# princeton-computational-imaging/Neural-Volume-Super-Resolution

Hardware: AMD Instinct MI355X
Metric: rendered rays/sec (64+128 samples) at 800x800 Lego-like view (higher is better)
Workload: dtype f32 as 2 f16 limbs (3 MFMA products, f32 acc); 1 GPU; Blender-'lego'-like 800x800 view, 64 coarse + 128 fine samples, tri-plane decoder (3x800^2x48 + 32^2x48 planes, 4+4x128 MLP), 1 view per GPU per step; partition=view

## Files before the change

include/nvsr.h:

```cpp
#ifndef NVSR_H
#define NVSR_H
#include <stdint.h>

#ifdef __cplusplus
extern "C" {
#endif

typedef void* nvsr_stream_t;

typedef enum {
    NVSR_OK = 0,
    NVSR_ERR_SHAPE = 1,
    NVSR_ERR_LAUNCH = 2,
    NVSR_ERR_NULL = 3,
    NVSR_ERR_ALIGN = 4
} nvsr_status;

#define NVSR_PLANE_CHANNELS 48
#define NVSR_DEC_CHANNELS 128
#define NVSR_DEC_LAYERS 4
#define NVSR_DECODER_NATURAL_FLOATS 130564
#define NVSR_DECODER_PACKED_F32_FLOATS 130576
#define NVSR_DECODER_PACKED_FLOATS 453136
#define NVSR_DECODER_PACKED_BWD_FLOATS 487424

typedef struct nvsr_scene {
    const float* planes[4];
    int32_t ph[4], pw[4];
    float lo[5];
    float range[5];
    float proj[3][6];
} nvsr_scene;

int nvsr_version(void);

#define NVSR_ARITH_INHERIT (-1)
#define NVSR_ARITH_INVALID (-2)
#define NVSR_ARITH_F32 0
#define NVSR_ARITH_F16 1
#define NVSR_ARITH_F16X2 2
#define NVSR_ARITH_BF16X3 3
#define NVSR_ARITH_DEFAULT NVSR_ARITH_F16X2
int nvsr_get_decoder_arithmetic(void);
int nvsr_set_decoder_arithmetic(int mode);
int nvsr_set_range_flag(uint32_t* device_word);
uint32_t* nvsr_get_range_flag(void);
int nvsr_release_render_scratch(void);
int64_t nvsr_render_scratch_bytes(void);
int nvsr_internal_group_order(const int* trips, int64_t G, int S, int* out, nvsr_stream_t stream);
int nvsr_internal_copy_group_order(int* dst, int64_t G, nvsr_stream_t stream);
int nvsr_internal_live_order(int* live_n, int64_t N, int S, nvsr_stream_t stream);
int nvsr_internal_colour_order_bins(void);
int nvsr_internal_copy_live_counts(int* dst, int64_t N, nvsr_stream_t stream);
int nvsr_internal_point_order(const int* entries, const float* lists, const float* rays, int64_t N, int S, int bands, int* points, int* steps, int* offsets,
                              nvsr_stream_t stream);
int nvsr_internal_point_bands(void);
int nvsr_internal_copy_point_steps(int* dst, int64_t G, nvsr_stream_t stream);
int64_t nvsr_occupancy_words(int G);
int64_t nvsr_occupancy_workspace_floats(int G, int K);
int nvsr_occupancy_build(const nvsr_scene* scene, const float* packed_decoder, int G, int K, float threshold, int dilate, int arithmetic, uint32_t* grid,
                         float* workspace, nvsr_stream_t stream);
int nvsr_render_pass_occupancy_arith(const nvsr_scene* scene, const float* packed_decoder, int64_t N, int S, const float* rays, const float* z, int lindisp,
                                     int white_bkgd, float* rgb, float* disp, float* acc, float* weights, float* depth, const uint32_t* grid, int G, int arithmetic,
                                     nvsr_stream_t stream);
int nvsr_render_rays_occupancy_arith(const nvsr_scene* scene, const float* packed_coarse, const float* packed_fine, int64_t N, int Nc, int Nf,
                                     const float* rays, int lindisp, int white_bkgd, const float* t_rand, const float* u, float* rgb_c, float* disp_c,
                                     float* acc_c, float* rgb_f, float* disp_f, float* acc_f, float* workspace, const uint32_t* grid_coarse, int G_coarse,
                                     const uint32_t* grid_fine, int G_fine, int arithmetic, nvsr_stream_t stream);
int nvsr_internal_occupancy_probes(const nvsr_scene* scene, int G, int K, float* x, nvsr_stream_t stream);
int nvsr_internal_occupancy_cull(const nvsr_scene* scene, int64_t N, int S, const float* rays, const float* z, int lindisp, const uint32_t* grid, int G, int* kept,
                                 int* kept_n, nvsr_stream_t stream);
int nvsr_internal_copy_kept_counts(int* dst, int64_t N, nvsr_stream_t stream);
int nvsr_limb_gemm_probe(int arithmetic, int K, const float* W, const float* X, float* Y, nvsr_stream_t stream);
#define NVSR_CONV_ARITH_DEFAULT NVSR_ARITH_F16X2
int nvsr_get_conv_arithmetic(void);
int nvsr_set_conv_arithmetic(int mode);

int nvsr_plane_to_channel_last(const float* nchw, float* nhwc, int C, int H, int W, nvsr_stream_t stream);
int nvsr_plane_from_channel_last(const float* nhwc, float* nchw, int C, int H, int W, nvsr_stream_t stream);

int nvsr_pack_decoder(const float* natural, float* packed, nvsr_stream_t stream);

int nvsr_get_ray_bundle(int H, int W, double focal_x, double focal_y, const float* c2w, int padding, double offset,
                        float* ro, float* rd, nvsr_stream_t stream);
int nvsr_get_ray_bundle_at(int H, int W, double focal_x, double focal_y, const float* c2w, double offset, int64_t N, const int32_t* row_col,
                           float* ro, float* rd, nvsr_stream_t stream);
int nvsr_sample_pixels(int64_t total, int H, int W, uint64_t key, int64_t first, int64_t n, const float* image, int channels,
                       int32_t* row_col, float* target, nvsr_stream_t stream);
uint64_t nvsr_sample_key(uint64_t seed, uint64_t calls);
int nvsr_sample_pixels_seq(int64_t total, int H, int W, uint64_t* state, int64_t first, int64_t n, const float* image, int channels,
                           int32_t* row_col, float* target, nvsr_stream_t stream);
#define NVSR_MSE_PAIR_MAX_ELEMS (1 << 22)
int nvsr_mse_pair(int64_t n, const float* a, const float* b, const float* target, float* losses, float* g_a, float* g_b, nvsr_stream_t stream);
int nvsr_mse_pair_sum(int64_t n, const float* a, const float* b, const float* target, float* losses3, nvsr_stream_t stream);
int nvsr_mse_pair_backward(int64_t n, const float* a, const float* b, const float* target, const float* scale_a, const float* scale_b, float* g_a,
                           float* g_b, nvsr_stream_t stream);
int nvsr_ndc_rays(int H, int W, double focal, double near_, int64_t N, const float* ro, const float* rd, float* ro_out,
                  float* rd_out, nvsr_stream_t stream);
int nvsr_pack_rays(int64_t N, const float* ro, const float* rd, const float* view_src, double near_, double far_,
                   float* rays, nvsr_stream_t stream);
int nvsr_coarse_z(int64_t N, int Nc, const float* rays, int lindisp, const float* t_rand, float* z, nvsr_stream_t stream);

int nvsr_sample_pdf(int64_t N, int nb, int ns, const float* bins, const float* weights, const float* u, float* samples,
                    nvsr_stream_t stream);
int nvsr_cumprod_exclusive(int64_t N, int n, const float* in, float* out, nvsr_stream_t stream);
int nvsr_cumprod_exclusive_backward(int64_t N, int n, const float* in, const float* out, const float* g_out, float* g_in,
                                    nvsr_stream_t stream);
int nvsr_sort_rows(int64_t N, int n, const float* in, float* out, nvsr_stream_t stream);
int nvsr_importance_resample(int64_t N, int Nc, int Nf, const float* z_coarse, const float* weights, const float* u,
                             float* z_fine, nvsr_stream_t stream);

int nvsr_importance_resample_rays(int64_t N, int Nc, int Nf, const float* rays, int lindisp, const float* weights, const float* u,
                                  float* z_fine, nvsr_stream_t stream);

int nvsr_triplane_decode(const nvsr_scene* scene, const float* packed_decoder, int64_t P, const float* x, float* out,
                         nvsr_stream_t stream);
int nvsr_triplane_decode_arith(const nvsr_scene* scene, const float* packed_decoder, int64_t P, const float* x, float* out, int arithmetic,
                               nvsr_stream_t stream);

int nvsr_composite(int64_t N, int S, const float* raw, const float* z, const float* rd, const float* noise, int white_bkgd,
                   float* rgb, float* disp, float* acc, float* weights, float* depth, nvsr_stream_t stream);

int nvsr_composite_mip(int64_t N, int S, const float* raw, const float* z, const float* rd, const float* noise, int white_bkgd,
                       float* rgb, float* disp, float* acc, float* weights , float* depth ,
                       nvsr_stream_t stream);
int nvsr_composite_rays(int64_t N, int S, const float* raw, const float* z, const float* rays, const float* noise, int white_bkgd,
                        float* rgb, float* disp, float* acc, float* weights, float* depth, nvsr_stream_t stream);

int nvsr_render_pass(const nvsr_scene* scene, const float* packed_decoder, int64_t N, int S, const float* rays, const float* z,
                     const float* noise, int white_bkgd, float* rgb, float* disp, float* acc, float* weights, float* depth,
                     nvsr_stream_t stream);

int nvsr_decode_rays(const nvsr_scene* scene, const float* packed_decoder, int64_t N, int S, const float* rays, const float* z,
                     float* raw, nvsr_stream_t stream);

#define NVSR_FUSED_MIN_RAYS 65536
int64_t nvsr_fused_min_rays(void);
int64_t nvsr_render_workspace_floats(int64_t N, int Nc, int Nf);
int nvsr_render_rays(const nvsr_scene* scene, const float* packed_coarse, const float* packed_fine, int64_t N, int Nc, int Nf,
// ... 275 lines not shown
```

neural-volume-super-resolution_amd/capi.py:

```python
import ctypes as C
import os

import torch

from .build import LIB_PATH as _DEFAULT_LIB_PATH

LIB_PATH = os.environ.get("NVSR_HIP_LIB", _DEFAULT_LIB_PATH)

PLANE_CHANNELS = 48
DEC_CHANNELS = 128
DECODER_NATURAL_FLOATS = 130564
DECODER_PACKED_FLOATS = 453136
DECODER_PACKED_BWD_FLOATS = 487424
MIP_NERF_NATURAL_FLOATS = 81092
MIP_NERF_RECORD_FLOATS = 767
MIP_NERF_GRAD_RECORD_FLOATS = 708
PE_NERF_NATURAL_FLOATS = 81476
PE_NERF_RECORD_FLOATS = 770
PE_NERF_GRAD_RECORD_FLOATS = 708
MSE_PAIR_MAX_ELEMS = 1 << 22

_STATUS = {1: "NVSR_ERR_SHAPE (argument out of the supported range)", 2: "NVSR_ERR_LAUNCH (kernel launch failed)",
           3: "NVSR_ERR_NULL (required pointer is NULL)", 4: "NVSR_ERR_ALIGN (pointer not 16-byte aligned)"}

# ... 78 lines not shown
    "nvsr_conv3x3_packed_floats": ([_i, _i], _i64),
    "nvsr_pack_conv3x3": ([_vp, _i, _i, _vp, _vp], _i),
    "nvsr_conv3x3": ([_vp, _i, _i, _i, _vp, _i, _i, _vp, _vp, _vp], _i),
    "nvsr_edsr_natural_floats": ([_i, _i, _i, _i, _i], _i64),
    "nvsr_edsr_packed_floats": ([_i, _i, _i, _i, _i], _i64),
    "nvsr_pack_edsr": ([_vp, _i, _i, _i, _i, _i, _vp, _vp], _i),
    "nvsr_pack_edsr_arith": ([_vp, _i, _i, _i, _i, _i, _vp, _i, _vp], _i),
    "nvsr_edsr_out_size": ([_i, _i, _i, _i, _ip, _ip], _i),
    "nvsr_edsr_workspace_floats": ([_i, _i, _i, _i, _i], _i64),
    "nvsr_edsr_forward": ([_vp, _i, _i, _i, _vp, _i, _i, _i, _i, _vp, _vp, _vp], _i),
    "nvsr_planes_sr_workspace_floats": ([_i, _i, _i, _i, _i, _i, _i, _fp], _i64),
    "nvsr_planes_sr": ([_vp, _i, _i, _i, _vp, _i, _i, _i, _i, _i, _fp, _vp, _vp, _vp, _vp, _vp], _i),
    "nvsr_render_pass_ex": ([C.POINTER(Scene), _vp, _i64, _i, _vp, _vp, _vp, _i, _vp, _vp, _vp, _vp, _vp, _vp, _vp], _i),
    "nvsr_pack_decoder_bwd": ([_vp, _vp, _vp], _i),
    "nvsr_composite_backward": ([_i64, _i, _vp, _vp, _vp, _vp, _i, _vp, _vp, _vp, _vp], _i),
    "nvsr_composite_backward_mip": ([_i64, _i, _vp, _vp, _vp, _vp, _i, _vp, _vp, _vp, _vp], _i),
    "nvsr_composite_backward_depth": ([_i64, _i, _vp, _vp, _vp, _vp, _i, _vp, _vp, _vp, _i, _vp, _vp], _i),
    "nvsr_composite_backward_rays": ([_i64, _i, _vp, _vp, _vp, _vp, _i, _vp, _vp, _vp, _i, _vp, _vp], _i),
    "nvsr_render_pass_backward": ([C.POINTER(Scene), _vp, _vp, _i64, _i, _vp, _vp, _vp, C.POINTER(C.c_void_p), _vp], _i),
    "nvsr_decode_rays_ex": ([C.POINTER(Scene), _vp, _i64, _i, _vp, _vp, _vp, _vp, _vp, _vp], _i),
    "nvsr_render_pass_backward_gates": ([C.POINTER(Scene), _vp, _vp, _i64, _i, _vp, _vp, _vp, _vp, C.POINTER(C.c_void_p), _vp, _vp, _vp], _i),
    "nvsr_view_grad_workspace_floats": ([_i64, _i], _i64),
    "nvsr_decoder_record_floats": ([_i64, _i], _i64),
    "nvsr_render_pass_backward_ex": ([C.POINTER(Scene), _vp, _vp, _i64, _i, _vp, _vp, _vp, C.POINTER(C.c_void_p), _vp, _vp, _vp], _i),
    "nvsr_decoder_weight_grad": ([_i64, _i, _vp, _vp, _vp], _i),
    "nvsr_edsr_forward_batch": ([_vp, _i, _i, _i, _i, _vp, _i, _i, _i, _i, _vp, _vp, _vp], _i),
    "nvsr_planes_sr_batch": ([C.POINTER(C.c_void_p), _i, _i, _i, _i, _vp, _i, _i, _i, _i, _i, _fp, _vp, _vp, C.POINTER(C.c_void_p), _vp, _vp], _i),
    "nvsr_pack_conv3x3_dgrad": ([_vp, _i, _i, _vp, _vp], _i),
    "nvsr_conv3x3_dgrad": ([_vp, _i, _i, _i, _vp, _i, _vp, _vp], _i),
    "nvsr_conv3x3_wgrad_workspace_floats": ([_i, _i, _i, _i], _i64),
    "nvsr_conv3x3_wgrad": ([_vp, _vp, _i, _i, _i, _i, C.c_float, _vp, _vp, _vp], _i),
    "nvsr_edsr_acts_floats": ([_i, _i, _i, _i, _i, _i, _i], _i64),
    "nvsr_edsr_forward_train": ([_vp, _i, _i, _i, _vp, _i, _i, _i, _i, _vp, _vp, _vp], _i),
    "nvsr_edsr_packed_dgrad_floats": ([_i, _i, _i, _i, _i], _i64),
    "nvsr_pack_edsr_dgrad": ([_vp, _i, _i, _i, _i, _i, _vp, _vp], _i),
    "nvsr_pack_edsr_dgrad_arith": ([_vp, _i, _i, _i, _i, _i, _vp, _i, _vp], _i),
    "nvsr_edsr_backward_workspace_floats": ([_i, _i, _i, _i, _i, _i, _i], _i64),
    "nvsr_edsr_backward": ([_vp, _i, _i, _i, _vp, _vp, _i, _i, _i, _i, _vp, _vp, _vp, _vp, _vp], _i),
    "nvsr_planes_sr_keep_floats": ([_i, _i, _i, _i, _i, _i, _i, _fp], _i64),
    "nvsr_planes_sr_train": ([_vp, _i, _i, _i, _vp, _i, _i, _i, _i, _i, _fp, _vp, _vp, _vp, _vp, _vp, _vp], _i),
    "nvsr_planes_sr_backward_workspace_floats": ([_i, _i, _i, _i, _i, _i, _i, _fp], _i64),
    "nvsr_planes_sr_backward": ([_i, _i, _i, _vp, _vp, _i, _i, _i, _i, _i, _fp, _vp, _vp, _vp, _vp, _vp, _vp], _i),
    "nvsr_generic_decoder_natural_floats": ([C.POINTER(DecoderGeometry)], _i64),
    "nvsr_generic_decode_workspace_floats": ([C.POINTER(DecoderGeometry), _i64], _i64),
    "nvsr_generic_decode": ([C.POINTER(Scene), C.POINTER(DecoderGeometry), _vp, _i64, _vp, _vp, _vp, _vp], _i),
    "nvsr_generic_decode_backward_workspace_floats": ([C.POINTER(DecoderGeometry), _i64], _i64),
    "nvsr_generic_decode_backward": ([C.POINTER(Scene), C.POINTER(DecoderGeometry), _vp, _i64, _vp, _vp, _vp, _vp, _vp, _vp, _vp, _vp, _vp], _i),
    "nvsr_generic_decoder_natural_floats_ext": ([C.POINTER(DecoderGeometry), _i], _i64),
    "nvsr_generic_decode_workspace_floats_ext": ([C.POINTER(DecoderGeometry), _i, _i64], _i64),
    "nvsr_generic_decode_backward_workspace_floats_ext": ([C.POINTER(DecoderGeometry), _i, _i64], _i64),
    "nvsr_generic_decode_ext": ([C.POINTER(SceneExt), C.POINTER(DecoderGeometry), _vp, _i64, _vp, _vp, _vp, _vp, _vp], _i),
    "nvsr_generic_fused_supported": ([C.POINTER(DecoderGeometry), _i], _i),
    "nvsr_generic_decode_fused_ext": ([C.POINTER(SceneExt), C.POINTER(DecoderGeometry), _vp, _i64, _vp, _vp, _vp, _vp], _i),
    "nvsr_generic_packed_floats_ext": ([C.POINTER(DecoderGeometry), _i], _i64),
    "nvsr_pack_generic_decoder_ext": ([C.POINTER(DecoderGeometry), _i, _vp, _vp, _vp], _i),
    "nvsr_generic_fused_supported_arith": ([C.POINTER(DecoderGeometry), _i, _i], _i),
    "nvsr_generic_decode_fused_arith_ext": ([C.POINTER(SceneExt), C.POINTER(DecoderGeometry), _vp, _vp, _i64, _vp, _vp, _vp, _i, _vp], _i),
    "nvsr_generic_decode_fused_density_arith_ext": ([C.POINTER(SceneExt), C.POINTER(DecoderGeometry), _vp, _vp, _i64, _vp, _vp, _vp, _i, _vp], _i),
    "nvsr_generic_decode_fused_colour_arith_ext": ([C.POINTER(SceneExt), C.POINTER(DecoderGeometry), _vp, _vp, _i64, _vp, _vp, _vp, _vp, _i64, _vp, _i,
                                                    _vp], _i),
    "nvsr_generic_live_list_workspace_bytes": ([_i64], _i64),
    "nvsr_generic_live_list": ([_i64, _vp, _vp, _vp, _vp, _vp], _i),
    "nvsr_generic_occupancy_build_ext": ([C.POINTER(SceneExt), C.POINTER(DecoderGeometry), _vp, _vp, _i, _i, C.c_float, _i, _i, _vp, _vp, _vp], _i),
    "nvsr_generic_occupancy_keep": ([C.POINTER(SceneExt), _i64, _vp, _vp, _i, _vp, _vp, _vp], _i),
    "nvsr_generic_decode_fused_density_list_arith_ext": ([C.POINTER(SceneExt), C.POINTER(DecoderGeometry), _vp, _vp, _i64, _vp, _vp, _vp, _vp, _i64, _vp,
                                                          _i, _vp], _i),
    "nvsr_generic_decode_backward_ext": ([C.POINTER(SceneExt), C.POINTER(DecoderGeometry), _vp, _i64, _vp, _vp, _vp, _vp, C.POINTER(C.c_void_p),
                                          _vp, _vp], _i),
    "nvsr_generic_backward_fused_supported": ([C.POINTER(DecoderGeometry), _i], _i),
    "nvsr_generic_decode_backward_fused_ext": ([C.POINTER(SceneExt), C.POINTER(DecoderGeometry), _vp, _i64, _vp, _vp, _vp, C.POINTER(C.c_void_p),
                                                _vp], _i),
    "nvsr_ray_points": ([_i64, _i, _vp, _vp, _vp, _vp], _i),
    "nvsr_render_shared_workspace_floats": ([_i64, _i, _i], _i64),
    "nvsr_render_rays_shared_arith": ([C.POINTER(Scene), _vp, _i64, _i, _i, _vp, _i, _i, _vp, _vp, _vp, _vp, _vp, _vp, _vp, _vp, _vp, _vp, _vp, _i, _vp], _i),
    "nvsr_shared_merge": ([_i64, _i, _i, _vp, _i, _vp, _vp, _vp, _vp, _vp, _vp], _i),
    "nvsr_release_render_scratch": ([], _i),
    "nvsr_render_scratch_bytes": ([], _i64),
    "nvsr_internal_group_order": ([_vp, _i64, _i, _vp, _vp], _i),
    "nvsr_internal_copy_group_order": ([_vp, _i64, _vp], _i),
    "nvsr_internal_live_order": ([_vp, _i64, _i, _vp], _i),
    "nvsr_internal_colour_order_bins": ([], _i),
    "nvsr_internal_copy_live_counts": ([_vp, _i64, _vp], _i),
    "nvsr_internal_point_bands": ([], _i),
    "nvsr_internal_copy_point_steps": ([_vp, _i64, _vp], _i),
    "nvsr_internal_point_order": ([_vp, _vp, _vp, _i64, _i, _i, _vp, _vp, _vp, _vp], _i),
    "nvsr_occupancy_words": ([_i], _i64),
    "nvsr_occupancy_workspace_floats": ([_i, _i], _i64),
    "nvsr_occupancy_build": ([C.POINTER(Scene), _vp, _i, _i, C.c_float, _i, _i, _vp, _vp, _vp], _i),
    "nvsr_render_pass_occupancy_arith": ([C.POINTER(Scene), _vp, _i64, _i, _vp, _vp, _i, _i, _vp, _vp, _vp, _vp, _vp, _vp, _i, _i, _vp], _i),
    "nvsr_render_rays_occupancy_arith": ([C.POINTER(Scene), _vp, _vp, _i64, _i, _i, _vp, _i, _i, _vp, _vp, _vp, _vp, _vp, _vp, _vp, _vp, _vp, _vp, _i, _vp, _i,
                                          _i, _vp], _i),
    "nvsr_internal_occupancy_probes": ([C.POINTER(Scene), _i, _i, _vp, _vp], _i),
    "nvsr_internal_occupancy_cull": ([C.POINTER(Scene), _i64, _i, _vp, _vp, _i, _vp, _i, _vp, _vp, _vp], _i),
    "nvsr_internal_copy_kept_counts": ([_vp, _i64, _vp], _i),
    "nvsr_set_sr_plane_interp": ([_i], _i),
    "nvsr_get_sr_plane_interp": ([], _i),
    "nvsr_set_sr_align_corners": ([_i], _i),
    "nvsr_get_sr_align_corners": ([], _i),
    "nvsr_render_pass_arith": ([C.POINTER(Scene), _vp, _i64, _i, _vp, _vp, _vp, _i, _vp, _vp, _vp, _vp, _vp, _vp, _i, _vp], _i),
    "nvsr_decode_rays_arith": ([C.POINTER(Scene), _vp, _i64, _i, _vp, _vp, _vp, _vp, _vp, _i, _vp], _i),
    "nvsr_render_rays_arith": ([C.POINTER(Scene), _vp, _vp, _i64, _i, _i, _vp, _i, _i, _vp, _vp, _vp, _vp, _vp, _vp, _vp, _vp, _vp,
                                _vp, _vp, _i, _vp], _i),
    "nvsr_render_pass_backward_gates_arith": ([C.POINTER(Scene), _vp, _vp, _i64, _i, _vp, _vp, _vp, _vp, C.POINTER(C.c_void_p), _vp, _vp, _i, _vp], _i),
    "nvsr_decoder_weight_grad_arith": ([_i64, _i, _vp, _vp, _i, _vp], _i),
    "nvsr_conv3x3_arith": ([_vp, _i, _i, _i, _vp, _i, _i, _vp, _vp, _i, _i, _vp], _i),
    "nvsr_conv3x3_dgrad_arith": ([_vp, _i, _i, _i, _vp, _i, _vp, _i, _i, _vp], _i),
    "nvsr_conv3x3_wgrad_arith": ([_vp, _vp, _i, _i, _i, _i, C.c_float, _vp, _vp, _i, _vp], _i),
    "nvsr_edsr_forward_batch_arith": ([_vp, _i, _i, _i, _i, _vp, _i, _i, _i, _i, _vp, _vp, _i, _vp], _i),
    "nvsr_edsr_forward_train_arith": ([_vp, _i, _i, _i, _vp, _i, _i, _i, _i, _vp, _vp, _i, _vp], _i),
    "nvsr_edsr_backward_arith": ([_vp, _i, _i, _i, _vp, _vp, _i, _i, _i, _i, _vp, _vp, _vp, _vp, _i, _vp], _i),
    "nvsr_planes_sr_arith": ([_vp, _i, _i, _i, _vp, _i, _i, _i, _i, _i, _fp, _vp, _vp, _vp, _vp, _i, _vp], _i),
    "nvsr_planes_sr_batch_arith": ([C.POINTER(C.c_void_p), _i, _i, _i, _i, _vp, _i, _i, _i, _i, _i, _fp, _vp, _vp, C.POINTER(C.c_void_p), _vp, _i, _vp], _i),
    "nvsr_planes_sr_train_arith": ([_vp, _i, _i, _i, _vp, _i, _i, _i, _i, _i, _fp, _vp, _vp, _vp, _vp, _vp, _i, _vp], _i),
    "nvsr_planes_sr_backward_arith": ([_i, _i, _i, _vp, _vp, _i, _i, _i, _i, _i, _fp, _vp, _vp, _vp, _vp, _vp, _i, _vp], _i),
    "nvsr_planes_sr_batch_ex": ([C.POINTER(C.c_void_p), _i, _i, _i, _i, _vp, _i, _i, _i, _i, _i, _fp, _vp, _vp, C.POINTER(C.c_void_p), _vp, _i, _i, _i, _vp], _i),
    "nvsr_planes_sr_batch_keep_floats": ([_i, _i, _i, _i, _i, _i, _i, _i, _fp], _i64),
    "nvsr_planes_sr_batch_workspace_floats": ([_i, _i, _i, _i, _i, _i, _i, _i, _fp], _i64),
    "nvsr_planes_sr_batch_backward_workspace_floats": ([_i, _i, _i, _i, _i, _i, _i, _i, _fp], _i64),
    "nvsr_planes_sr_train_batch_arith": ([C.POINTER(C.c_void_p), _i, _i, _i, _i, _vp, _i, _i, _i, _i, _i, _fp, _vp, _vp, C.POINTER(C.c_void_p), _vp, _vp,
                                          _i, _i, _i, _vp], _i),
    "nvsr_planes_sr_backward_batch_arith": ([_i, _i, _i, _i, _vp, _vp, _i, _i, _i, _i, _i, _fp, _vp, C.POINTER(C.c_void_p), _vp, C.POINTER(C.c_void_p), _vp,
                                             _i, _i, _i, _vp], _i),
    "nvsr_planes_sr_backward_batch_marks": ([_i, _i, _i, _i, _vp, _vp, _i, _i, _i, _i, _i, _fp, _vp, C.POINTER(C.c_void_p), _vp, C.POINTER(C.c_void_p), _vp,
                                             _i, _i, _i, _i, C.POINTER(C.c_int32), C.POINTER(C.c_void_p), _vp], _i),
    "nvsr_positional_encoding": ([_i64, _i, _vp, _i, _i, _vp, _vp], _i),
    "nvsr_flexible_nerf_forward": ([_i64, _vp, _i, _i, _i, _i, _i, _vp, _vp, _vp], _i),
    "nvsr_mip_encode": ([_i64, _i, _vp, _vp, _d, _vp, _vp], _i),
    "nvsr_mip_nerf_forward_arith": ([_i64, _i, _vp, _vp, _d, _vp, _vp, _vp, _i, _vp], _i),
    "nvsr_mip_nerf_backward_arith": ([_i64, _vp, _vp, _vp, _vp, _i, _vp], _i),
    "nvsr_mip_nerf_wgrad_workspace_floats": ([_i64], _i64),
    "nvsr_mip_nerf_weight_grad": ([_i64, _vp, _vp, _vp, _vp, _vp], _i),
    "nvsr_pe_encode": ([_i64, _i, _vp, _vp, _vp, _vp], _i),
    "nvsr_pe_nerf_forward_arith": ([_i64, _i, _vp, _vp, _vp, _vp, _vp, _i, _vp], _i),
    "nvsr_pe_nerf_backward_arith": ([_i64, _vp, _vp, _vp, _vp, _i, _vp], _i),
    "nvsr_pe_nerf_wgrad_workspace_floats": ([_i64], _i64),
    "nvsr_pe_nerf_weight_grad": ([_i64, _vp, _vp, _vp, _vp, _vp], _i),
    "nvsr_render_pass_backward_rows_arith": ([C.POINTER(Scene), _vp, _vp, _i64, _i, _vp, _vp, _vp, _vp, C.POINTER(C.c_void_p), _vp, _vp, _i, _vp], _i),
    "nvsr_view_rows_reduce": ([_i64, _i, _vp, _vp, _vp], _i),
    "nvsr_internal_plane_taps": ([C.POINTER(Scene), _i, _i64, _i, _vp, _vp, _vp, _vp, _vp], _i),
    "nvsr_rows_scatter_workspace_bytes": ([_i64], _i64),
    "nvsr_rows_scatter": ([_i64, _vp, _vp, _vp, _i, _i, _vp, _vp, _i64, _vp], _i),
    "nvsr_decoder_weight_grad_det_workspace_floats": ([_i64, _i], _i64),
    "nvsr_decoder_weight_grad_det_arith": ([_i64, _i, _vp, _vp, _vp, _i, _vp], _i),
    "nvsr_lowrank_planes": ([LowrankPlanesArgs, _vp], _i),
    "nvsr_lowrank_planes_backward": ([LowrankPlanesArgs, _vp], _i),
}

_PROTOS_LAUNCH = {
    "nvsr_render_pass2_launch": ([C.POINTER(Scene), _vp, _i64, _i, _vp, _vp, _vp, _i, _vp, _vp, _vp, _vp, _vp, _vp, _vp], _i),
    "nvsr_render_pass3_launch": ([_i, C.POINTER(Scene), _vp, _i64, _i, _vp, _vp, _vp, _i, _vp, _vp, _vp, _vp, _vp, _vp, _vp], _i),
    "nvsr_render_pass3_coarse_z_launch": ([_i, C.POINTER(Scene), _vp, _i64, _i, _vp, _i, _vp, _i, _vp, _vp, _vp, _vp, _vp, _vp, _vp], _i),
    "nvsr_decode_rays_limb_launch": ([_i, C.POINTER(Scene), _vp, _i64, _i, _vp, _vp, _vp, _vp, _vp, _vp], _i),
    "nvsr_decode_rays_pair_launch": ([C.POINTER(Scene), _vp, _i64, _i, _vp, _vp, _vp, _vp, _vp], _i),
    "nvsr_internal_conv_route": ([_i, _i, _i, _i, _i, _i, _ip, _ip, C.POINTER(C.c_uint)], _i),
}

_lib = None


ARITHMETIC = {"f32": 0, "f16x2": 2, "bf16x3": 3}
CONV_ARITHMETIC = {**ARITHMETIC, "f16": 1}
RENDER_ARITHMETIC = {**ARITHMETIC, "f16": 1}
SR_BATCH_MAX = 4
ARITH_INHERIT = -1


# ... 194 lines not shown
```

neural-volume-super-resolution_amd/csrc/colour_order.h:

```cpp
#pragma once
#include "tile_pair.h"

namespace nvsr {

constexpr int ORDER_SHIFT = 12, ORDER_RAYS = 1 << ORDER_SHIFT, ORDER_BINS = 32;
constexpr int ORDER_MAX_S = 1 << (31 - ORDER_SHIFT);
static_assert(ORDER_RAYS % RAYS2 == 0, "a block of the ray order is a whole number of workgroups");

#ifndef NVSR_POINT_BANDS
#define NVSR_POINT_BANDS 0
#endif
constexpr int POINT_BANDS = NVSR_POINT_BANDS, POINT_NONE = -1, POINT_VIEW_FLOATS = 2 * HALF_C;
static_assert(RAYS2 <= 256 && ORDER_MAX_S <= (1 << 24), "a slot and a list index share an entry");

struct LiveLists { float* z; float* w; int* n; int* slot; int* trip; int* pts; int* steps; float* views; };

struct KeptLists { int* idx; int* n; int* slot; int* trip; };

enum class PassRoute { Fused, TwoPhase, Occupancy };
PassRoute acquire_pass_scratch(int64_t N, int S, hipStream_t stream, bool raw_out, bool want_kept, bool launch, LiveLists& live, KeptLists& kept);
void launch_colour_order(const LiveLists& ll, int64_t N, int S, hipStream_t stream);
void launch_kept_order(const KeptLists& kl, int64_t N, int S, hipStream_t stream);
void launch_point_order(const LiveLists& ll, const float* rays_nf, int64_t N, int S, hipStream_t stream);

}
```

neural-volume-super-resolution_amd/csrc/colour_order.hip:

```cpp
#include "colour_order.h"
#include "occupancy.h"
#include "nvsr_internal.h"

#include <cstdlib>
#include <mutex>
#include <vector>

namespace nvsr {

constexpr int SORT_TPB = 1024, SORT_WAVES = SORT_TPB / 64, SORT_ROUNDS = 4, SORT_MAX = SORT_TPB * SORT_ROUNDS;
template <int NKEYS>
__device__ __forceinline__ void counting_sort(const int (&key)[SORT_ROUNDS], int nkeys, int n, int (&start)[SORT_ROUNDS], int (&place)[SORT_ROUNDS],
                                              int (&len)[SORT_ROUNDS]) {
    static_assert(NKEYS <= SORT_TPB, "one thread per key sums the tables");
    __shared__ int cnt_s[NKEYS * SORT_WAVES];
    __shared__ int tot_s[NKEYS], start_s[NKEYS];
    const int wave = threadIdx.x >> 6, lane = threadIdx.x & 63;
    const unsigned long long below = (1ull << lane) - 1ull;
    for (int b = 0; b <= nkeys; ++b) {
        int c = 0;
#pragma unroll
        for (int r = 0; r < SORT_ROUNDS; ++r) c += __popcll(__ballot(key[r] == b));
        if (lane == 0) cnt_s[b * SORT_WAVES + wave] = c;
    }
    __syncthreads();
    if ((int)threadIdx.x <= nkeys) {
        int run = 0;
        for (int w = 0; w < SORT_WAVES; ++w) { const int c = cnt_s[threadIdx.x * SORT_WAVES + w]; cnt_s[threadIdx.x * SORT_WAVES + w] = run; run += c; }
        tot_s[threadIdx.x] = run;
    }
    __syncthreads();
    if ((int)threadIdx.x <= nkeys) {
        int run = 0;
        for (int b = nkeys; b > (int)threadIdx.x; --b) run += tot_s[b];
        start_s[threadIdx.x] = run;
    }
    __syncthreads();
#pragma unroll
    for (int r = 0; r < SORT_ROUNDS; ++r) start[r] = place[r] = len[r] = 0;
    if (wave * (64 * SORT_ROUNDS) >= n) return;
    for (int b = 0; b <= nkeys; ++b) {
        int at = cnt_s[b * SORT_WAVES + wave];
#pragma unroll
        for (int r = 0; r < SORT_ROUNDS; ++r) {
            const unsigned long long m = __ballot(key[r] == b);
            if (key[r] == b) place[r] = at + __popcll(m & below);
            at += __popcll(m);
        }
    }
#pragma unroll
    for (int r = 0; r < SORT_ROUNDS; ++r)
        if (key[r] >= 0) { start[r] = start_s[key[r]]; len[r] = tot_s[key[r]]; }
}

static_assert(ORDER_RAYS == SORT_MAX && SORT_WAVES == ORDER_RAYS / RAYS2 && RAYS2 % 64 == 0, "one block of the order per sort, one wave of it per colour workgroup");
__global__ __launch_bounds__(SORT_TPB) void live_order_kernel(int* __restrict__ live_n, long N, int S, int bins, int* __restrict__ group_trip) {
    __shared__ int out_s[ORDER_RAYS];
    const long block_base = (long)blockIdx.x * ORDER_RAYS;
    const int M = (int)(N - block_base < ORDER_RAYS ? N - block_base : ORDER_RAYS);
    const int wave = threadIdx.x >> 6, lane = threadIdx.x & 63;
    int cnt[SORT_ROUNDS], bin[SORT_ROUNDS];
#pragma unroll
    for (int r = 0; r < SORT_ROUNDS; ++r) {
        const int i = wave * (64 * SORT_ROUNDS) + r * 64 + lane;
        cnt[r] = i < M ? live_n[block_base + i] : 0;
        const int b = (int)(((unsigned)cnt[r] * (unsigned)bins + (unsigned)(S - 1)) / (unsigned)S);
        bin[r] = i < M ? (b < bins ? b : bins) : -1;
    }
    int start[SORT_ROUNDS], place[SORT_ROUNDS], len[SORT_ROUNDS];
    counting_sort<ORDER_BINS + 1>(bin, bins, M, start, place, len);
#pragma unroll
    for (int r = 0; r < SORT_ROUNDS; ++r)
        if (bin[r] >= 0) out_s[start[r] + place[r]] = (cnt[r] << ORDER_SHIFT) | (wave * (64 * SORT_ROUNDS) + r * 64 + lane);
    __syncthreads();
#pragma unroll
    for (int r = 0; r < SORT_ROUNDS; ++r) {
        const int i = threadIdx.x + r * SORT_TPB;
        if (i < M) live_n[block_base + i] = out_s[i];
    }
    if (group_trip && wave * RAYS2 < M) {
        int m = 0;
#pragma unroll
        for (int r = 0; r < RAYS2 / 64; ++r) {
            const int i = wave * RAYS2 + r * 64 + lane;
            if (i < M) m = max(m, out_s[i] >> ORDER_SHIFT);
        }
#pragma unroll
        for (int o = 32; o >= 1; o >>= 1) m = max(m, __shfl_xor(m, o));
        if (lane == 0) group_trip[(long)blockIdx.x * SORT_WAVES + wave] = m;
    }
}

constexpr int GORDER_MAX_G = SORT_MAX, GORDER_MAX_S = 511;
__global__ __launch_bounds__(SORT_TPB) void group_order_kernel(const int* __restrict__ group_trip, int G, int S, int sorted, int* __restrict__ group_slot) {
    if (!sorted || G > GORDER_MAX_G || S > GORDER_MAX_S) {
        const unsigned per = (unsigned)G >> 3, rem = (unsigned)G & 7u;
        for (unsigned r = threadIdx.x; r < (unsigned)G; r += SORT_TPB) {
            const unsigned xcd = r & 7u;
            group_slot[r] = (int)(xcd * per + (xcd < rem ? xcd : rem) + (r >> 3));
        }
        return;
    }
    const int wave = threadIdx.x >> 6, lane = threadIdx.x & 63;
    int key[SORT_ROUNDS];
#pragma unroll
    for (int r = 0; r < SORT_ROUNDS; ++r) {
        const int g = wave * (64 * SORT_ROUNDS) + r * 64 + lane;
        const int t = g < G ? group_trip[g] : 0;
        key[r] = g < G ? (t < 0 ? 0 : t > S ? S : t) : -1;
    }
    int start[SORT_ROUNDS], place[SORT_ROUNDS], len[SORT_ROUNDS];
    counting_sort<GORDER_MAX_S + 1>(key, S, G, start, place, len);
#pragma unroll
    for (int r = 0; r < SORT_ROUNDS; ++r) {
        if (key[r] < 0) continue;
        const int run = len[r], per = run >> 3, rem = run & 7, thr = rem * (per + 1);
        const int j = place[r];
        const int k = j < thr ? j / (per + 1) : rem + (j - thr) / (per ? per : 1);
        const int i = j < thr ? j - k * (per + 1) : (j - thr) - (k - rem) * per;
        group_slot[start[r] + k + 8 * i] = wave * (64 * SORT_ROUNDS) + r * 64 + lane;
    }
}

__global__ __launch_bounds__(RAYS2) void point_order_kernel(const int* __restrict__ live_n, const float* __restrict__ live_z, const float* __restrict__ rays_nf,
                                                            long N, int S, int nb, int* __restrict__ pts, int* __restrict__ steps, int* __restrict__ offs) {
    __shared__ int wsum_s[2][RAYS2 / 64], kmin_s[RAYS2], cnt_s[RAYS2], start_s[RAYS2], stage_s[RAYS2];
    const int j = threadIdx.x, wave = j >> 6, lane = j & 63;
    const long slot0 = (long)blockIdx.x * RAYS2;
    int n = 0;
    long ray = 0;
    if (slot0 + j < N) {
        const int e = live_n[slot0 + j];
        n = e >> ORDER_SHIFT;
        ray = slot0 / ORDER_RAYS * ORDER_RAYS + (e & (ORDER_RAYS - 1));
    }
    const float* lz = live_z + ray * S;
    const float nr = rays_nf ? rays_nf[ray * 11 + 6] : 0.0f, fr = rays_nf ? rays_nf[ray * 11 + 7] : 0.0f;
    auto band_of = [&](int k) -> int {
        const float e = lz[k];
        if (!rays_nf) {
            const long long b = (long long)__float_as_int(e) * nb / S;
            return b < 0 ? 0 : b < nb ? (int)b : nb - 1;
        }
        const float u = __fdiv_rn(__fmul_rn(__fsub_rn(e, nr), (float)nb), __fsub_rn(fr, nr));
        return u >= 0.0f ? (u < (float)nb ? (int)u : nb - 1) : 0;
    };
    auto scan = [&](int c, int buf, int& total) -> int {
        int incl = c;
#pragma unroll
        for (int o = 1; o < 64; o <<= 1) { const int v = __shfl_up(incl, o); if (lane >= o) incl += v; }
        if (lane == 63) wsum_s[buf][wave] = incl;
        __syncthreads();
        int before = 0;
        total = 0;
#pragma unroll
        for (int w = 0; w < RAYS2 / 64; ++w) { const int v = wsum_s[buf][w]; if (w < wave) before += v; total += v; }
        return before + incl - c;
    };
    int* out = pts + (long)blockIdx.x * RAYS2 * S;
    int k = 0, base = 0, nextb = n > 0 ? band_of(0) : nb;
    for (int b = 0; b < nb; ++b) {
        const int k0 = k;
        while (k < n && nextb <= b) { ++k; if (k < n) nextb = max(nextb, band_of(k)); }
        int total;
        const int at = base + scan(k - k0, b & 1, total);
        for (int i = k0; i < k; ++i) out[at + (i - k0)] = (j << 24) | i;
        base += total;
    }
    const int nsteps = (base + RAYS2 - 1) / RAYS2;
    if (base + j < nsteps * RAYS2) out[base + j] = POINT_NONE;
    if (j == 0) { steps[blockIdx.x] = nsteps; offs[blockIdx.x] = (int)blockIdx.x * S; }
    __syncthreads();
    for (int t = 0; t < nsteps; ++t) {
        const int e = out[t * RAYS2 + j];
        const bool valid = e != POINT_NONE;
        const int sl = (int)((unsigned)e >> 24), kk = e & 0xffffff;
        kmin_s[j] = 0x7fffffff; cnt_s[j] = 0;
        __syncthreads();
        if (valid) { atomicMin(&kmin_s[sl], kk); atomicAdd(&cnt_s[sl], 1); }
        __syncthreads();
        int total;
        start_s[j] = scan(cnt_s[j], 0, total);
        __syncthreads();
        stage_s[valid ? start_s[sl] + (kk - kmin_s[sl]) : j] = e;
        __syncthreads();
        out[t * RAYS2 + j] = stage_s[j];
    }
}

namespace {
enum { LISTS, GROUP, POINTS, VIEWS, KEPT, KEPT_GROUP, N_BUFFERS };
struct Buffer { void* p; size_t bytes; };
struct Launch { int64_t N; int* n; int* steps; int64_t kept_N; int* kept; };
struct Scratch { int device; hipStream_t stream; Buffer buf[N_BUFFERS]; Launch last; };
std::mutex g_live_mutex;
std::vector<Scratch> g_live;

Scratch* find_scratch(int device, hipStream_t stream) {
    for (Scratch& c : g_live)
        if (c.device == device && c.stream == stream) return &c;
    return nullptr;
}

bool grow(Scratch& e, int which, size_t bytes) {
    Buffer& b = e.buf[which];
    if (b.bytes >= bytes) return true;
    if (b.p) (void)hipFree(b.p);
    b = Buffer{};
    e.last = Launch{};
    void* p = nullptr;
    if (hipMalloc(&p, bytes) != hipSuccess) { (void)hipGetLastError(); return false; }
    b = Buffer{p, bytes};
    return true;
}

int64_t groups_of(int64_t N) { return (N + RAYS2 - 1) / RAYS2; }

template <class Pick>
int copy_left_behind(int* dst, int64_t ints, nvsr_stream_t stream, Pick pick) {
    if (!dst) return NVSR_ERR_NULL;
    int device = 0;
    if (hipGetDevice(&device) != hipSuccess) return NVSR_ERR_LAUNCH;
    const int* src = nullptr;
    {
        std::lock_guard<std::mutex> lock(g_live_mutex);
        const Scratch* c = find_scratch(device, (hipStream_t)stream);
        if (c) src = pick(*c);
    }
    if (!src) return NVSR_ERR_SHAPE;
    return hipMemcpyAsync(dst, src, (size_t)ints * sizeof(int), hipMemcpyDefault, (hipStream_t)stream) == hipSuccess ? NVSR_OK : NVSR_ERR_LAUNCH;
}

bool env_starts(const char* name, char c) {
    const char* e = getenv(name);
    return e && e[0] == c;
}
void launch_live_order(int* live_n, int64_t N, int S, int bins, int* group_trip, hipStream_t stream) {
    hipLaunchKernelGGL(live_order_kernel, dim3((unsigned)((N + ORDER_RAYS - 1) / ORDER_RAYS)), dim3(SORT_TPB), 0, stream, live_n, (long)N, S, bins, group_trip);
}
void launch_group_order(const int* group_trip, int64_t G, int S, int* group_slot, hipStream_t stream) {
    const int sorted = !env_starts("NVSR_COLOUR_GROUP_ORDER", '0');
    hipLaunchKernelGGL(group_order_kernel, dim3(1), dim3(SORT_TPB), 0, stream, group_trip, (int)G, S, sorted, group_slot);
}
void launch_point_order(const int* live_n, const float* live_z, const float* rays_nf, int64_t N, int S, int nb, int* pts, int* steps, int* offs, hipStream_t stream) {
    nb = nb < 1 || nb > S ? S : nb;
    hipLaunchKernelGGL(point_order_kernel, dim3((unsigned)groups_of(N)), dim3(RAYS2), 0, stream, live_n, live_z, rays_nf, (long)N, S, nb, pts, steps, offs);
}
}

PassRoute acquire_pass_scratch(int64_t N, int S, hipStream_t stream, bool raw_out, bool want_kept, bool launch, LiveLists& live, KeptLists& kept) {
    bool declines = raw_out || S < 1 || S >= ORDER_MAX_S || env_starts("NVSR_RENDER_ONE_PHASE", '1');
    if (!declines) {
        hipStreamCaptureStatus cap = hipStreamCaptureStatusNone;
        if (hipStreamIsCapturing(stream, &cap) != hipSuccess || cap != hipStreamCaptureStatusNone) { (void)hipGetLastError(); declines = true; }
    }
    if (declines && !want_kept) return PassRoute::Fused;
    int device = 0;
    if (hipGetDevice(&device) != hipSuccess) return PassRoute::Fused;
    const size_t rows = (size_t)N * (size_t)S, G = (size_t)groups_of(N);
    std::lock_guard<std::mutex> lock(g_live_mutex);
    Scratch* e = find_scratch(device, stream);
    if (e && want_kept) { e->last.kept_N = 0; e->last.kept = nullptr; }
    if (declines) return PassRoute::Fused;
    if (!e) {
        g_live.emplace_back();
        e = &g_live.back();
        e->device = device; e->stream = stream;
    }
    if (!grow(*e, GROUP, 2 * G * sizeof(int)) || !grow(*e, LISTS, (2 * rows + (size_t)N) * sizeof(float)) || !e->buf[LISTS].p) return PassRoute::Fused;
    live = LiveLists{};
    live.z = static_cast<float*>(e->buf[LISTS].p);
    live.w = live.z + rows;
    live.n = reinterpret_cast<int*>(live.w + rows);
    live.slot = static_cast<int*>(e->buf[GROUP].p);
    live.trip = live.slot + G;
    const size_t npts = G * RAYS2 * (size_t)S;
    if (!env_starts("NVSR_COLOUR_POINTS", '0') && G * (size_t)S <= 0x7fffffffu && grow(*e, POINTS, (npts + 2 * G) * sizeof(int)) &&
        grow(*e, VIEWS, G * RAYS2 * POINT_VIEW_FLOATS * sizeof(float))) {
        live.pts = static_cast<int*>(e->buf[POINTS].p);
        live.steps = live.pts + npts;
        live.views = static_cast<float*>(e->buf[VIEWS].p);
    }
    PassRoute route = PassRoute::TwoPhase;
    if (want_kept && grow(*e, KEPT_GROUP, 2 * G * sizeof(int)) && grow(*e, KEPT, (rows + (size_t)N) * sizeof(int))) {
        kept.idx = static_cast<int*>(e->buf[KEPT].p);
        kept.n = kept.idx + rows;
        kept.slot = static_cast<int*>(e->buf[KEPT_GROUP].p);
        kept.trip = kept.slot + G;
        route = PassRoute::Occupancy;
    }
    if (launch) e->last = route == PassRoute::Occupancy ? Launch{N, live.n, live.steps, N, kept.n} : Launch{N, live.n, live.steps, e->last.kept_N, e->last.kept};
    return route;
}

static void launch_orders(int* n, int* trip, int* slot, int64_t N, int S, hipStream_t stream) {
    launch_live_order(n, N, S, env_starts("NVSR_COLOUR_ORDER", '0') ? 0 : ORDER_BINS, trip, stream);
    launch_group_order(trip, groups_of(N), S, slot, stream);
}
void launch_kept_order(const KeptLists& kl, int64_t N, int S, hipStream_t stream) { launch_orders(kl.n, kl.trip, kl.slot, N, S, stream); }
void launch_colour_order(const LiveLists& ll, int64_t N, int S, hipStream_t stream) { launch_orders(ll.n, ll.trip, ll.slot, N, S, stream); }

void launch_point_order(const LiveLists& ll, const float* rays_nf, int64_t N, int S, hipStream_t stream) {
    launch_point_order(ll.n, ll.z, rays_nf, N, S, POINT_BANDS, ll.pts, ll.steps, ll.steps + groups_of(N), stream);
}

}

using namespace nvsr;

extern "C" int nvsr_internal_colour_order_bins(void) { return ORDER_BINS; }
extern "C" int nvsr_internal_live_order(int* live_n, int64_t N, int S, nvsr_stream_t stream) {
    if (!live_n) return NVSR_ERR_NULL;
    if (N < 1 || S < 1 || S >= ORDER_MAX_S || (N + ORDER_RAYS - 1) / ORDER_RAYS > 0x7fffffff) return NVSR_ERR_SHAPE;
    launch_live_order(live_n, N, S, ORDER_BINS, nullptr, (hipStream_t)stream);
    return NVSR_CHECK_LAUNCH();
}
extern "C" int nvsr_internal_copy_live_counts(int* dst, int64_t N, nvsr_stream_t stream) {
    return copy_left_behind(dst, N, stream, [N](const Scratch& c) { return c.last.N == N ? c.last.n : nullptr; });
}
extern "C" int nvsr_internal_group_order(const int* trips, int64_t G, int S, int* out, nvsr_stream_t stream) {
    if (!trips || !out) return NVSR_ERR_NULL;
    if (G < 1 || G > 0x7fffffff || S < 1 || S >= ORDER_MAX_S) return NVSR_ERR_SHAPE;
    launch_group_order(trips, G, S, out, (hipStream_t)stream);
    return NVSR_CHECK_LAUNCH();
}
extern "C" int nvsr_internal_copy_group_order(int* dst, int64_t G, nvsr_stream_t stream) {
    return copy_left_behind(dst, 2 * G, stream, [G](const Scratch& c) { return c.last.n && groups_of(c.last.N) == G ? static_cast<int*>(c.buf[GROUP].p) : nullptr; });
}

extern "C" int nvsr_internal_point_bands(void) { return POINT_BANDS; }
extern "C" int nvsr_internal_point_order(const int* entries, const float* lists, const float* rays, int64_t N, int S, int bands, int* points, int* steps, int* offsets,
                                         nvsr_stream_t stream) {
    if (!entries || !lists || !points || !steps || !offsets) return NVSR_ERR_NULL;
    const int64_t G = (N + RAYS2 - 1) / RAYS2;
    if (N < 1 || S < 1 || S >= ORDER_MAX_S || G * S > 0x7fffffff) return NVSR_ERR_SHAPE;
    launch_point_order(entries, lists, rays, N, S, bands, points, steps, offsets, (hipStream_t)stream);
    return NVSR_CHECK_LAUNCH();
}
extern "C" int nvsr_internal_copy_point_steps(int* dst, int64_t G, nvsr_stream_t stream) {
    return copy_left_behind(dst, G, stream, [G](const Scratch& c) { return c.last.n && groups_of(c.last.N) == G ? c.last.steps : nullptr; });
}

extern "C" int nvsr_internal_copy_kept_counts(int* dst, int64_t N, nvsr_stream_t stream) {
    return copy_left_behind(dst, N, stream, [N](const Scratch& c) { return c.last.kept_N == N ? c.last.kept : nullptr; });
}

extern "C" void nvsr_internal_reserve_render_scratch(int64_t N, int S, nvsr_stream_t stream) {
    LiveLists live;
    KeptLists kept;
    (void)acquire_pass_scratch(N, S, (hipStream_t)stream,  false,  false,  false, live, kept);
}

extern "C" int64_t nvsr_render_scratch_bytes(void) {
    std::lock_guard<std::mutex> lock(g_live_mutex);
    int64_t total = 0;
    for (const Scratch& c : g_live) total += (int64_t)c.buf[LISTS].bytes;
    return total;
}

extern "C" int nvsr_release_render_scratch(void) {
    std::lock_guard<std::mutex> lock(g_live_mutex);
    int prev = 0;
    const bool have_prev = hipGetDevice(&prev) == hipSuccess;
    int rc = NVSR_OK;
    for (const Scratch& c : g_live)
        for (const Buffer& b : c.buf)
            if (b.p && (hipSetDevice(c.device) != hipSuccess || hipFree(b.p) != hipSuccess)) rc = NVSR_ERR_LAUNCH;
    g_live.clear();
    if (have_prev) (void)hipSetDevice(prev);
    return rc;
}
```

Baseline: 8.289 million rays/s.

## Build point order with a single-pass per-band count sweep kernel

Adds a point_sweep_kernel that counts each ray's points per depth band into byte counters in shared memory and scans them with DPP wave scans. It then emits the point ordering in one sweep across the bands instead of running the original point_order_kernel's iterative scan and stage loop. It is templated on the row count and is chosen by default when S<=255, with an environment variable to turn it off. This is meant to cut the cost of the reordering step that runs before decoding, in exchange for more shared memory per block and a second, harder-to-verify code path.

Result: no change. 8.364 million rays/s (median of 6 runs) (+0.9%).

```diff
diff --git a/include/nvsr.h b/include/nvsr.h
--- a/include/nvsr.h
+++ b/include/nvsr.h
@@ -55,6 +55,7 @@
 int nvsr_internal_point_order(const int* entries, const float* lists, const float* rays, int64_t N, int S, int bands, int* points, int* steps, int* offsets,
                               nvsr_stream_t stream);
 int nvsr_internal_point_bands(void);
+int nvsr_internal_point_order_sweeps(int S);
 int nvsr_internal_copy_point_steps(int* dst, int64_t G, nvsr_stream_t stream);
 int64_t nvsr_occupancy_words(int G);
 int64_t nvsr_occupancy_workspace_floats(int G, int K);
diff --git a/neural-volume-super-resolution_amd/capi.py b/neural-volume-super-resolution_amd/capi.py
--- a/neural-volume-super-resolution_amd/capi.py
+++ b/neural-volume-super-resolution_amd/capi.py
@@ -184,6 +184,7 @@
     "nvsr_internal_colour_order_bins": ([], _i),
     "nvsr_internal_copy_live_counts": ([_vp, _i64, _vp], _i),
     "nvsr_internal_point_bands": ([], _i),
+    "nvsr_internal_point_order_sweeps": ([_i], _i),
     "nvsr_internal_copy_point_steps": ([_vp, _i64, _vp], _i),
     "nvsr_internal_point_order": ([_vp, _vp, _vp, _i64, _i, _i, _vp, _vp, _vp, _vp], _i),
     "nvsr_occupancy_words": ([_i], _i64),
diff --git a/neural-volume-super-resolution_amd/csrc/colour_order.h b/neural-volume-super-resolution_amd/csrc/colour_order.h
--- a/neural-volume-super-resolution_amd/csrc/colour_order.h
+++ b/neural-volume-super-resolution_amd/csrc/colour_order.h
@@ -13,6 +13,33 @@
 constexpr int POINT_BANDS = NVSR_POINT_BANDS, POINT_NONE = -1, POINT_VIEW_FLOATS = 2 * HALF_C;
 static_assert(RAYS2 <= 256 && ORDER_MAX_S <= (1 << 24), "a slot and a list index share an entry");
 
+constexpr int SWEEP_MAX_S = 255;
+struct SweepStep { int t, below, mine, kmin; };
+__host__ __device__ inline void sweep_take(SweepStep& s, int lo, int hi, int at, int c, int k0) {
+    const int below = (at < hi ? at : hi) - lo;
+    if (below > 0) s.below += below;
+    const int first = at > lo ? at : lo, last = at + c < hi ? at + c : hi;
+    if (last > first) {
+        if (!s.mine) s.kmin = k0 + (first - at);
+        s.mine += last - first;
+    }
+}
+__host__ __device__ inline void sweep_emit(SweepStep& s, int j, int* out) {
+    for (int i = 0; i < s.mine; ++i) out[s.t * RAYS2 + s.below + i] = (j << 24) | (s.kmin + i);
+    s = SweepStep{s.t + 1, 0, 0, 0};
+}
+__host__ __device__ inline void sweep_band(SweepStep& s, int j, int base, int total, int at, int c, int k0, int* out) {
+    int lo = base;
+    const int end = base + total;
+    while (end >= (s.t + 1) * RAYS2) {
+        const int edge = (s.t + 1) * RAYS2;
+        sweep_take(s, lo, edge, at, c, k0);
+        sweep_emit(s, j, out);
+        lo = edge;
+    }
+    sweep_take(s, lo, end, at, c, k0);
+}
+
 struct LiveLists { float* z; float* w; int* n; int* slot; int* trip; int* pts; int* steps; float* views; };
 
 struct KeptLists { int* idx; int* n; int* slot; int* trip; };
diff --git a/neural-volume-super-resolution_amd/csrc/colour_order.hip b/neural-volume-super-resolution_amd/csrc/colour_order.hip
--- a/neural-volume-super-resolution_amd/csrc/colour_order.hip
+++ b/neural-volume-super-resolution_amd/csrc/colour_order.hip
@@ -1,6 +1,7 @@
 #include "colour_order.h"
 #include "occupancy.h"
 #include "nvsr_internal.h"
+#include "wave_scan.h"
 
 #include <cstdlib>
 #include <mutex>
@@ -122,29 +123,97 @@
     }
 }
 
+struct SlotList { int n; const float* lz; float nr, fr; };
+__device__ __forceinline__ SlotList slot_list(const int* __restrict__ live_n, const float* __restrict__ live_z, const float* __restrict__ rays_nf, long N, int S, long slot) {
+    int n = 0;
+    long ray = 0;
+    if (slot < N) {
+        const int e = live_n[slot];
+        n = e >> ORDER_SHIFT;
+        ray = slot / ORDER_RAYS * ORDER_RAYS + (e & (ORDER_RAYS - 1));
+    }
+    return SlotList{n, live_z + ray * S, rays_nf ? rays_nf[ray * 11 + 6] : 0.0f, rays_nf ? rays_nf[ray * 11 + 7] : 0.0f};
+}
+__device__ __forceinline__ int point_band(float e, bool depths, float nr, float fr, int nb, int S) {
+    if (!depths) {
+        const int s = __float_as_int(e);
+        return s < 0 ? 0 : s >= S ? nb - 1 : nb == S ? s : (int)((long long)s * nb / S);
+    }
+    const float u = __fdiv_rn(__fmul_rn(__fsub_rn(e, nr), (float)nb), __fsub_rn(fr, nr));
+    return u >= 0.0f ? (u < (float)nb ? (int)u : nb - 1) : 0;
+}
+
+template <int CTRL, int ROW_MASK>
+__device__ __forceinline__ int dpp_or_zero(int v) { return __builtin_amdgcn_update_dpp(0, v, CTRL, ROW_MASK, 0xf, false); }
+__device__ __forceinline__ int wave_scan_count(int v) {
+    v += dpp_or_zero<DPP_ROW_SHR1, 0xf>(v);
+    v += dpp_or_zero<DPP_ROW_SHR2, 0xf>(v);
+    v += dpp_or_zero<DPP_ROW_SHR4, 0xf>(v);
+    v += dpp_or_zero<DPP_ROW_SHR8, 0xf>(v);
+    v += dpp_or_zero<DPP_ROW_BCAST15, 0xa>(v);
+    v += dpp_or_zero<DPP_ROW_BCAST31, 0xc>(v);
+    return v;
+}
+
+constexpr int SWEEP_LOADS = 16;
+template <int ROWS>
+__global__ __launch_bounds__(RAYS2) void point_sweep_kernel(const int* __restrict__ live_n, const float* __restrict__ live_z, const float* __restrict__ rays_nf,
+                                                            long N, int S, int nb, int* __restrict__ pts, int* __restrict__ steps, int* __restrict__ offs) {
+    static_assert(ROWS <= SWEEP_MAX_S && RAYS2 == 4 * 64, "a byte per count; four wave totals per band");
+    __shared__ __attribute__((aligned(16))) unsigned cnt_s[ROWS * (RAYS2 / 4)];
+    NVSR_RACE_PROBE_DELAY(cnt_s);
+    __shared__ __attribute__((aligned(16))) int wtot_s[ROWS][RAYS2 / 64];
+    const int j = threadIdx.x, wave = j >> 6, lane = j & 63;
+    const SlotList sl = slot_list(live_n, live_z, rays_nf, N, S, (long)blockIdx.x * RAYS2 + j);
+    const int n = sl.n;
+    unsigned char* col = reinterpret_cast<unsigned char*>(cnt_s) + j;
+    for (int b = 0; b < nb; ++b) col[b * RAYS2] = 0;
+    int cur = 0, run = 0;
+    for (int k0 = 0; k0 < n; k0 += SWEEP_LOADS) {
+        float e[SWEEP_LOADS];
+#pragma unroll
+        for (int u = 0; u < SWEEP_LOADS; ++u) e[u] = sl.lz[min(k0 + u, n - 1)];
+#pragma unroll
+        for (int u = 0; u < SWEEP_LOADS; ++u) {
+            if (k0 + u >= n) break;
+            const int b = max(cur, point_band(e[u], rays_nf != nullptr, sl.nr, sl.fr, nb, S));
+            if (b != cur) { col[cur * RAYS2] = (unsigned char)run; cur = b; run = 0; }
+            ++run;
+        }
+    }
+    col[cur * RAYS2] = (unsigned char)run;
+    for (int b = 0; b < nb; ++b) {
+        const int c = col[b * RAYS2];
+        const int incl = __ballot(c != 0) ? wave_scan_count(c) : 0;
+        if (lane == 63) wtot_s[b][wave] = incl;
+    }
+    __syncthreads();
+    int* out = pts + (long)blockIdx.x * RAYS2 * S;
+    int base = 0, k = 0;
+    SweepStep step{0, 0, 0, 0};
+    for (int b = 0; b < nb; ++b) {
+        const int4 w = *reinterpret_cast<const int4*>(wtot_s[b]);
+        const int before = (wave > 0 ? w.x : 0) + (wave > 1 ? w.y : 0) + (wave > 2 ? w.z : 0), total = w.x + w.y + w.z + w.w;
+        if (total == 0) continue;
+        const int c = col[b * RAYS2];
+        const int incl = wave_scan_count(c);
+        sweep_band(step, j, base, total, base + before + incl - c, c, k, out);
+        base += total;
+        k += c;
+    }
+    const int nsteps = (base + RAYS2 - 1) / RAYS2;
+    if (step.t < nsteps) sweep_emit(step, j, out);
+    if (base + j < nsteps * RAYS2) out[base + j] = POINT_NONE;
+    if (j == 0) { steps[blockIdx.x] = nsteps; offs[blockIdx.x] = (int)blockIdx.x * S; }
+}
+
 __global__ __launch_bounds__(RAYS2) void point_order_kernel(const int* __restrict__ live_n, const float* __restrict__ live_z, const float* __restrict__ rays_nf,
                                                             long N, int S, int nb, int* __restrict__ pts, int* __restrict__ steps, int* __restrict__ offs) {
     __shared__ int wsum_s[2][RAYS2 / 64], kmin_s[RAYS2], cnt_s[RAYS2], start_s[RAYS2], stage_s[RAYS2];
     const int j = threadIdx.x, wave = j >> 6, lane = j & 63;
-    const long slot0 = (long)blockIdx.x * RAYS2;
-    int n = 0;
-    long ray = 0;
-    if (slot0 + j < N) {
-        const int e = live_n[slot0 + j];
-        n = e >> ORDER_SHIFT;
-        ray = slot0 / ORDER_RAYS * ORDER_RAYS + (e & (ORDER_RAYS - 1));
-    }
-    const float* lz = live_z + ray * S;
-    const float nr = rays_nf ? rays_nf[ray * 11 + 6] : 0.0f, fr = rays_nf ? rays_nf[ray * 11 + 7] : 0.0f;
-    auto band_of = [&](int k) -> int {
-        const float e = lz[k];
-        if (!rays_nf) {
-            const long long b = (long long)__float_as_int(e) * nb / S;
-            return b < 0 ? 0 : b < nb ? (int)b : nb - 1;
-        }
-        const float u = __fdiv_rn(__fmul_rn(__fsub_rn(e, nr), (float)nb), __fsub_rn(fr, nr));
-        return u >= 0.0f ? (u < (float)nb ? (int)u : nb - 1) : 0;
-    };
+    const SlotList sl = slot_list(live_n, live_z, rays_nf, N, S, (long)blockIdx.x * RAYS2 + j);
+    const int n = sl.n;
+    auto band_of = [&](int k) -> int { return point_band(sl.lz[k], rays_nf != nullptr, sl.nr, sl.fr, nb, S); };
     auto scan = [&](int c, int buf, int& total) -> int {
         int incl = c;
 #pragma unroll
@@ -242,9 +311,14 @@
     const int sorted = !env_starts("NVSR_COLOUR_GROUP_ORDER", '0');
     hipLaunchKernelGGL(group_order_kernel, dim3(1), dim3(SORT_TPB), 0, stream, group_trip, (int)G, S, sorted, group_slot);
 }
+bool point_order_sweeps(int S) { return S <= SWEEP_MAX_S && !env_starts("NVSR_POINT_ORDER_SWEEP", '0'); }
 void launch_point_order(const int* live_n, const float* live_z, const float* rays_nf, int64_t N, int S, int nb, int* pts, int* steps, int* offs, hipStream_t stream) {
     nb = nb < 1 || nb > S ? S : nb;
-    hipLaunchKernelGGL(point_order_kernel, dim3((unsigned)groups_of(N)), dim3(RAYS2), 0, stream, live_n, live_z, rays_nf, (long)N, S, nb, pts, steps, offs);
+    const dim3 grid((unsigned)groups_of(N)), block(RAYS2);
+    if (!point_order_sweeps(S)) hipLaunchKernelGGL(point_order_kernel, grid, block, 0, stream, live_n, live_z, rays_nf, (long)N, S, nb, pts, steps, offs);
+    else if (S <= 64) hipLaunchKernelGGL(point_sweep_kernel<64>, grid, block, 0, stream, live_n, live_z, rays_nf, (long)N, S, nb, pts, steps, offs);
+    else if (S <= 192) hipLaunchKernelGGL(point_sweep_kernel<192>, grid, block, 0, stream, live_n, live_z, rays_nf, (long)N, S, nb, pts, steps, offs);
+    else hipLaunchKernelGGL(point_sweep_kernel<SWEEP_MAX_S>, grid, block, 0, stream, live_n, live_z, rays_nf, (long)N, S, nb, pts, steps, offs);
 }
 }
 
@@ -329,6 +403,7 @@
 }
 
 extern "C" int nvsr_internal_point_bands(void) { return POINT_BANDS; }
+extern "C" int nvsr_internal_point_order_sweeps(int S) { return point_order_sweeps(S) ? 1 : 0; }
 extern "C" int nvsr_internal_point_order(const int* entries, const float* lists, const float* rays, int64_t N, int S, int bands, int* points, int* steps, int* offsets,
                                          nvsr_stream_t stream) {
     if (!entries || !lists || !points || !steps || !offsets) return NVSR_ERR_NULL;
```
